# gpcv-liujin/Deep3D_Aerial

Hardware: AMD Instinct MI355X
Metric: cost-volume Mvoxels/s (5v x 384D) (higher is better)
Workload: dtype f32; 1 GPU; config 2: fused homography-warp + variance, 5 views x 384 planes, features 32x688x464 fp32 (2752x1856 image at 1/4 res), one reference view per step per GPU

## Files before the change

### deep3d_aerial_amd/csrc/planesweep_tiled.hip

```cpp
#include "common.h"

#include <hip/hip_fp16.h>

#include "sweep_params.h"
#include "sweep_device.h"

#include <cstdlib>

namespace d3d {

namespace {

constexpr int TW = 32;
#ifndef D3D_NSUB
#define D3D_NSUB 4
#endif
#ifndef D3D_NLOADW
#define D3D_NLOADW 4
#endif
constexpr int DEFAULT_NSUB = D3D_NSUB;
constexpr int DEFAULT_NLOADW = D3D_NLOADW;
constexpr int DEFAULT_NPIXW = 2;
constexpr int DSEG_MAX = 128;
constexpr int MAXSTEPS = 64;
constexpr int PFD = 2;
constexpr int LDS_PIPE = 1;
constexpr int NCAND = 4;
constexpr int MAXRECTS = 512;
constexpr int RING_RW_QUANT = 8;
constexpr int RING_RH_QUANT = 2;
template <int STRIDE>
__host__ __device__ __forceinline__ int ring_row_floats(int RW) {
    const int n = (RW + 1) * STRIDE;
    return ((n - 32 + 63) & ~63) + 32;
}

#ifdef D3D_EXPERIMENTS
#define D3D_STAMPS 1
#else
#define D3D_STAMPS 0
#endif
#define D3D_CLOCK() (D3D_STAMPS ? clock64() : 0ll)

struct TiledArgs {
    int ngroups;
    int dseg;
    int cap_floats;
    int nseg;
    int tiles_x, tiles_y;
    int tall;
    const float* cl;
    unsigned long long* tstats;
    unsigned* stats;
};

template <int CW, int NSRC>
struct Lds {
    static constexpr int STRIDE = CW + 4;
    static constexpr int ZERO = 0;
    static constexpr int PMIN = 2 * STRIDE;
    static constexpr int PMAX = PMIN + DSEG_MAX;
    static constexpr int HDR = PMAX + DSEG_MAX;
    static constexpr int VT = HDR + 32;
    static constexpr int PLAN = VT + 8 * NSRC;
    static constexpr int SST = PLAN + MAXSTEPS * NSRC * 8;
    static constexpr int STOT = SST + MAXSTEPS + 4;
    static constexpr int RECTS = ((STOT + MAXSTEPS + 3) / 4) * 4;
    static constexpr int DATA = RECTS + (MAXRECTS + 1) * 4;
};

__device__ __forceinline__ int posmod(int a, int n) {
    int r = a % n;
    return r < 0 ? r + n : r;
}


struct RingView {
    int RW, RH;
    int rowb;
    int base;
};

template <int STRIDE>
__device__ __forceinline__ TapL geo_ring(const Ray& r, float tx, float ty, float tz, float d, float umax, float vmax, int kx, int ky,
                                         const RingView& R) {
    const float px = __fadd_rn(__fmul_rn(r.rx, d), tx);
    const float py = __fadd_rn(__fmul_rn(r.ry, d), ty);
    const float pz = __fadd_rn(__fmul_rn(r.rz, d), tz);
    const float iz = __builtin_amdgcn_rcpf(pz);
    const float u0 = px * iz, v0 = py * iz;
    float u = fmaf(fmaf(-u0, pz, px), iz, u0);
    float v = fmaf(fmaf(-v0, pz, py), iz, v0);
    u = __builtin_amdgcn_fmed3f(u, -1.0f, umax);
    v = __builtin_amdgcn_fmed3f(v, -1.0f, vmax);
    const float fu = floorf(u), fv = floorf(v);
    const float ax = u - fu, ay = v - fv;
    const float bx = (fu + 1.0f) - u, by = (fv + 1.0f) - v;
    TapL t;
    t.nw = bx * by;
    t.ne = ax * by;
    t.sw = bx * ay;
// ... 238 lines not shown
                vmin = fminf(vmin, v); vmax = fmaxf(vmax, v);
            }
            int wx0 = max((int)floorf(umin - 0.0625f), -1);
            int wy0 = max((int)floorf(vmin - 0.0625f), -1);
            int wx1 = min((int)floorf(umax + 0.0625f) + 1, w + 1);
            int wy1 = min((int)floorf(vmax + 0.0625f) + 1, h + 1);
            int ww = max(wx1 - wx0 + 1, 0), wh = max(wy1 - wy0 + 1, 0);
            if (vsel >= p.n_src) { wx0 = -1; wy0 = -1; ww = 2; wh = 2; ok = true; }
            if (!act) { ww = 0; wh = 0; ok = true; }
            int ux = ww, uy = wh;
            {
                const int qx0 = __shfl_up(wx0, 1), qy0 = __shfl_up(wy0, 1);
                const int qw = __shfl_up(ww, 1), qh = __shfl_up(wh, 1);
                if (lane > 0 && act && qw > 0 && ww > 0) {
                    ux = max(wx0 + ww, qx0 + qw) - min(wx0, qx0);
                    uy = max(wy0 + wh, qy0 + qh) - min(wy0, qy0);
                }
            }
            const int RWc = max(wave_maxi(ux), 1), RHc = max(wave_maxi(uy), 1);
            const int badc = (__any(!ok) || !feasible) ? 1 : 0;
            int* e = ldsi + CT + ((cand * NSRC + vsel) * 64 + lane) * 4;
            e[0] = wx0; e[1] = wy0; e[2] = ww; e[3] = wh;
            if (lane == 0) {
                int* hd = ldsi + CHD + (cand * NSRC + vsel) * 4;
                hd[0] = RWc; hd[1] = RHc; hd[2] = badc; hd[3] = nstepc;
            }
        }
    };
    constexpr int NCAND1 = NCAND - 1;
    for (int wk = wave; wk < NCAND1 * NSRC; wk += NWAVES) candidate_windows(wk / NSRC, wk % NSRC);
    __syncthreads();
    const long long t_p1 = D3D_CLOCK();
    auto plan_tables = [&](int cbeg, int cend) {
        int mode = 0, sp_sel = NSUB, nsteps_sel = (nplanes + NSUB - 1) / NSUB;
        for (int cand = cbeg; cand < cend && !mode; ++cand) {
            const int nsteps = ldsi[CHD + (cand * NSRC) * 4 + 3];
            const bool act = lane < nsteps;
            int wx0[NSRC], wy0[NSRC], ww[NSRC], wh[NSRC], RW[NSRC], RH[NSRC];
            int bad = 0, total = 0, totalq = 0;
            int RWq[NSRC], RHq[NSRC];
#pragma unroll
            for (int i = 0; i < NSRC; ++i) {
                const int* hd = ldsi + CHD + (cand * NSRC + i) * 4;
                RW[i] = hd[0]; RH[i] = hd[1]; bad |= hd[2];
                RWq[i] = (RW[i] + RING_RW_QUANT - 1) / RING_RW_QUANT * RING_RW_QUANT;
                RHq[i] = (RH[i] + RING_RH_QUANT - 1) / RING_RH_QUANT * RING_RH_QUANT;
                total += ring_row_floats<STRIDE>(RW[i]) * (RH[i] + 1);
                totalq += ring_row_floats<STRIDE>(RWq[i]) * (RHq[i] + 1);
            }
            if (totalq <= a.cap_floats) {
                total = totalq;
#pragma unroll
                for (int i = 0; i < NSRC; ++i) { RW[i] = RWq[i]; RH[i] = RHq[i]; }
            }
            if (bad || total > a.cap_floats) continue;
#pragma unroll
            for (int i = 0; i < NSRC; ++i) {
                const int* e = ldsi + CT + ((cand * NSRC + i) * 64 + lane) * 4;
                wx0[i] = e[0]; wy0[i] = e[1]; ww[i] = e[2]; wh[i] = e[3];
            }
            if (!bad && total <= a.cap_floats) {
                mode = 1;
                sp_sel = cand_planes(cand);
                nsteps_sel = nsteps;
                int base = L::DATA;
                int oxv[NSRC], oyv[NSRC], basev[NSRC];
                bool dims_ok = true;
#pragma unroll
                for (int i = 0; i < NSRC; ++i) {
                    const int cx0 = __shfl(wx0[i], 0), cy0 = __shfl(wy0[i], 0);
                    oxv[i] = posmod(wx0[i] - cx0, RW[i]);
                    oyv[i] = posmod(wy0[i] - cy0, RH[i]);
                    basev[i] = base;
                    dims_ok = dims_ok && RW[i] < 256 && RH[i] < 256;
                    if (act) {
                        int* e = ldsi + L::PLAN + (lane * NSRC + i) * 8;
                        e[0] = wx0[i]; e[1] = wy0[i]; e[2] = ww[i]; e[3] = wh[i];
                        e[4] = oxv[i];
                        e[5] = oyv[i];
                        e[6] = oxv[i] - wx0[i];
                        e[7] = oyv[i] - wy0[i];
                    }
                    if (lane == 0) {
                        ldsi[L::HDR + 4 + 4 * i + 0] = RW[i];
                        ldsi[L::HDR + 4 + 4 * i + 1] = RH[i];
                        ldsi[L::HDR + 4 + 4 * i + 2] = base;
                        ldsi[L::HDR + 4 + 4 * i + 3] = RW[i] | (RH[i] << 8) | ((base >> 2) << 16);
                        if constexpr (VIEW_MAJOR) {
                            const float* __restrict__ M = p.proj34 + 12 * min(i, p.n_src - 1);
                            const bool dummy = i >= p.n_src;
                            lds[L::VT + 8 * i + 0] = dummy ? -1.0f : M[3];
                            lds[L::VT + 8 * i + 1] = dummy ? -1.0f : M[7];
                            lds[L::VT + 8 * i + 2] = dummy ? 1.0f : M[11];
                            lds[L::VT + 8 * i + 3] = 0.0f;
                            ldsi[L::VT + 8 * i + 4] = RW[i];
                            ldsi[L::VT + 8 * i + 5] = RH[i];
                            ldsi[L::VT + 8 * i + 6] = ring_row_floats<STRIDE>(RW[i]) * 4;
                            ldsi[L::VT + 8 * i + 7] = lds_base_bytes(lds) + 4 * base;
                        }
                    }
                    base += ring_row_floats<STRIDE>(RW[i]) * (RH[i] + 1);
                }
                int cnt[NSRC][4], rx[NSRC][4], ry[NSRC][4], rwid[NSRC][4], nel[NSRC][4];
                int npos = 0;
#pragma unroll
                for (int i = 0; i < NSRC; ++i) {
                    const int xa = wx0[i], xb = wx0[i] + ww[i] - 1, ya = wy0[i], yb = wy0[i] + wh[i] - 1;
                    const int pxa = __shfl_up(wx0[i], 1), pya = __shfl_up(wy0[i], 1);
                    const int pxb = pxa + __shfl_up(ww[i], 1) - 1, pyb = pya + __shfl_up(wh[i], 1) - 1;
                    int ix0 = 1, ix1 = 0, iy0 = 1, iy1 = 0;
                    if (lane > 0) { ix0 = max(xa, pxa); ix1 = min(xb, pxb); iy0 = max(ya, pya); iy1 = min(yb, pyb); }
                    const bool ov = (ix0 <= ix1) && (iy0 <= iy1);
                    int rh_[4];
                    rx[i][0] = xa;      ry[i][0] = ya;      rwid[i][0] = (ov ? ix0 - 1 : xb) - xa + 1; rh_[0] = wh[i];
                    rx[i][1] = ix1 + 1; ry[i][1] = ya;      rwid[i][1] = ov ? xb - ix1 : 0;             rh_[1] = wh[i];
                    rx[i][2] = ix0;     ry[i][2] = ya;      rwid[i][2] = ov ? ix1 - ix0 + 1 : 0;        rh_[2] = ov ? iy0 - ya : 0;
                    rx[i][3] = ix0;     ry[i][3] = iy1 + 1; rwid[i][3] = ov ? ix1 - ix0 + 1 : 0;        rh_[3] = ov ? yb - iy1 : 0;
#pragma unroll
                    for (int r = 0; r < 4; ++r) {
                        nel[i][r] = act ? max(rwid[i][r], 0) * max(rh_[r], 0) : 0;
                        cnt[i][r] = (nel[i][r] + 63) >> 6;
                        npos += nel[i][r];
                    }
                }
                int nrect = 0;
#pragma unroll
                for (int i = 0; i < NSRC; ++i)
#pragma unroll
                    for (int r = 0; r < 4; ++r) nrect += cnt[i][r] > 0 ? 1 : 0;
                int incl = nrect;
#pragma unroll
                for (int sft = 1; sft < 64; sft <<= 1) {
                    int o = __shfl_up(incl, sft);
                    if (lane >= sft) incl += o;
                }
                const int total_rects = __shfl(incl, 63);
                if (total_rects > MAXRECTS || !dims_ok || __any(npos > 0xffff) || w > 0xfff0 || h > 0xfff0) {
                    mode = 0;
                } else {
                    int idx = incl - nrect;
                    if (act) ldsi[L::SST + lane] = idx;
                    if (lane == nsteps - 1) ldsi[L::SST + nsteps] = incl;
                    int pstart = 0;
#pragma unroll
                    for (int i = 0; i < NSRC; ++i)
#pragma unroll
                        for (int r = 0; r < 4; ++r)
                            if (cnt[i][r] > 0) {
                                int* e = ldsi + L::RECTS + 4 * idx;
                                e[0] = (rx[i][r] + 1) | ((ry[i][r] + 1) << 16);
                                e[1] = rwid[i][r] | (i << 12) | (pstart << 16);
                                e[2] = nel[i][r];
                                e[3] = (rx[i][r] - wx0[i] + oxv[i]) | ((ry[i][r] - wy0[i] + oyv[i]) << 16);
                                pstart += nel[i][r];
                                ++idx;
                            }
                    if (act) ldsi[L::STOT + lane] = pstart;
                }
            }
        }
        if (lane == 0) {
            ldsi[L::HDR + 0] = mode;
            ldsi[L::HDR + 1] = sp_sel;
            ldsi[L::HDR + 2] = nsteps_sel;
        }
    };
    if (wave == 0) plan_tables(0, NCAND1);
    __syncthreads();
    if (rfl(ldsi[L::HDR + 0]) == 0) {
        __syncthreads();
        for (int wk = wave; wk < NSRC; wk += NWAVES) candidate_windows(NCAND1, wk);
        __syncthreads();
        if (wave == 0) plan_tables(NCAND1, NCAND);
        __syncthreads();
    }
    if (D3D_STAMPS && a.tstats && tid == 0) {
        const long long t_p2 = clock64();
        atomicAdd(a.tstats + 16, (unsigned long long)(t_range - t_start));
        atomicAdd(a.tstats + 17, (unsigned long long)(t_p1 - t_range));
        atomicAdd(a.tstats + 18, (unsigned long long)(t_p2 - t_p1));
    }
    const int ring = rfl(ldsi[L::HDR + 0]);
    const int SP = rfl(ldsi[L::HDR + 1]);
    const int nsteps = rfl(ldsi[L::HDR + 2]);
    if (D3D_STAMPS && a.stats && tid == 0) {
        atomicAdd(a.stats + (ring ? 0 : 1), 1u);
        atomicAdd(a.stats + 2, (unsigned)SP);
        atomicAdd(a.stats + 3, (unsigned)nsteps);
        if (ring) {
            unsigned tot = 0;
            for (int i = 0; i < NSRC; ++i) tot += (ldsi[L::HDR + 4 + 4 * i] + 1) * (ldsi[L::HDR + 5 + 4 * i] + 1);
            atomicAdd(a.stats + 4, tot);
        }
    }
    struct Item {
        const float* g;
        int meta;
        int geo;
    };
    long long fdelta[NSRC];
#pragma unroll
    for (int i = 0; i < NSRC; ++i) {
        const long long d0 = reinterpret_cast<long long>(p.feats[1]);
        const long long di = reinterpret_cast<long long>(p.feats[i + 1]);
        fdelta[i] = (i < p.n_src) ? di - d0 : 0;
    }
    auto item = [&](int el, int Tn, int rb, const int (&pst16)[MAXRS]) -> Item {
        Item I;
        const bool live = el < Tn;
        int ridx = rb - 1;
#pragma unroll
        for (int rr = 0; rr < MAXRS; ++rr) ridx += (pst16[rr] <= el) ? 1 : 0;
        ridx = max(ridx, rb);
        const int* e = ldsi + L::RECTS + 4 * ridx;
        const int e0 = e[0], e1 = e[1], e6 = e[3];
        const int rx = (e0 & 0xffff) - 1, ry = (e0 >> 16) - 1;
        const int rwid = e1 & 0xfff, vi = (e1 >> 12) & 0xf, pst = (unsigned)e1 >> 16;
        const int e7 = ldsi[L::HDR + 4 + 4 * vi + 3];
        const int RWv = e7 & 0xff, RHv = (e7 >> 8) & 0xff, bs = (e7 >> 16) << 2;
        const int pos = el - pst;
        const int cy = (int)(((float)pos + 0.5f) * __builtin_amdgcn_rcpf((float)max(rwid, 1)));
        const int cx = pos - cy * rwid;
        const int sx = rx + cx, sy = ry + cy;
        const bool ok = live && ((unsigned)sx < (unsigned)w) && ((unsigned)sy < (unsigned)h);
        long long dsel = 0;
#pragma unroll
        for (int i = 1; i < NSRC; ++i) dsel = (vi == i) ? fdelta[i] : dsel;
        if (a.cl)
            I.g = a.cl + ((size_t)(vi * a.ngroups + grp) * plane + (size_t)(ok ? sy * w + sx : 0)) * CW;
        else
            I.g = reinterpret_cast<const float*>(reinterpret_cast<const char*>(p.feats[1]) + dsel) + (size_t)c0 * plane +
                  (ok ? sy * w + sx : 0);
        unsigned c = (unsigned)((e6 & 0xffff) + cx), r = (unsigned)((e6 >> 16) + cy);
        c = min(c, c - (unsigned)RWv);
        r = min(r, r - (unsigned)RHv);
        const int dst = bs + (int)r * ring_row_floats<STRIDE>(RWv) + (int)c * STRIDE;
        I.meta = live ? (dst | (ok ? 1 << 20 : 0) | (c == 0 ? 1 << 21 : 0) | (r == 0 ? 1 << 22 : 0)) : -1;
        I.geo = e7 & 0xffff;
        return I;
    };
    auto put = [&](int meta, int geo, int q, f4 v) {
        if (meta >= 0) {
            const int dst = (meta & 0xfffff) + 4 * q;
            const int RWv = geo & 0xff, RHv = geo >> 8;
            const int dupc = (meta >> 21) & 1 ? RWv * STRIDE : 0;
            const int dupr = (meta >> 22) & 1 ? RHv * ring_row_floats<STRIDE>(RWv) : 0;
            f4 x = (meta >> 20) & 1 ? v : (f4){0, 0, 0, 0};
            *reinterpret_cast<f4*>(lds + dst) = x;
            if (dupc) *reinterpret_cast<f4*>(lds + dst + dupc) = x;
            if (dupr) *reinterpret_cast<f4*>(lds + dst + dupr) = x;
            if (dupc && dupr) *reinterpret_cast<f4*>(lds + dst + dupc + dupr) = x;
        }
    };
    constexpr bool ONE_RECT = NPIXW <= 2;
    struct Rects {
        int psv, d0, d1, d3, d7;
    };
    const bool small32 = plane <= (size_t)0xffffffffu / (size_t)(CH * 4 > 64 ? CH * 4 : 64);
    f4 pf[PFD][Q];
    int pmeta[PFD], pgeo[PFD];
    int pkind[PFD];
    auto write_round = [&]() {
#pragma unroll
        for (int j = 0; j < PFD; ++j) {
            if (pkind[j] == 0) {
                if (pmeta[j] >= 0) {
#pragma unroll
                    for (int q = 0; q < Q; ++q) *reinterpret_cast<f4*>(lds + pmeta[j] + 4 * q) = pf[j][q];
                }
            } else {
#pragma unroll
                for (int q = 0; q < Q; ++q) put(pmeta[j], pgeo[j], q, pf[j][q]);
            }
        }
    };
    const bool ltiming = D3D_STAMPS && a.tstats != nullptr && lw == 0;
    long long lt_issue = 0, lt_write = 0, lt_bar = 0;
    auto stage = [&](int k, int sw, int snw) {
        const int rb = rfl(ldsi[L::SST + k]), re = rfl(ldsi[L::SST + k + 1]);
        const int Tn = rfl(ldsi[L::STOT + k]);
        const int nitems = (Tn + 63) >> 6;
        Rects R;
        {
            const bool have = lane < re - rb;
            const int* e = ldsi + L::RECTS + 4 * (rb + min(lane, MAXRS - 1));
            R.d1 = e[1];
            R.psv = have ? (int)((unsigned)R.d1 >> 16) : 0x7fffffff;
            if constexpr (ONE_RECT) {
                R.d0 = e[0]; R.d3 = e[3];
                R.d7 = ldsi[L::HDR + 4 + 4 * (have ? (R.d1 >> 12) & 0xf : 0) + 3];
            } else {
                R.d0 = R.d3 = R.d7 = 0;
            }
        }
        const int psv = R.psv;
        int pst16[MAXRS];
#pragma unroll
        for (int rr = 0; rr < MAXRS; ++rr) pst16[rr] = __builtin_amdgcn_readlane(psv, rr);
        unsigned n_items = 0, n_one = 0, n_plain = 0, n_in = 0, n_nodup = 0, n_idle = 0;
        for (int it0 = sw; it0 < nitems; it0 += snw * PFD) {
            long long tq1 = 0, tq2 = 0;
            if (ltiming) tq1 = clock64();
#pragma unroll
            for (int j = 0; j < PFD; ++j) {
                const int it = it0 + snw * j;
                int meta = -1, geo = 0, kind = 0;
                f4 v[Q];
                if (it < nitems) {
                    const int el0 = it * 64;
                    const int nlive = min(Tn - el0, 64);
                    const bool one = ONE_RECT && __ballot(psv > el0 && psv < el0 + nlive) == 0ull;
                    if (D3D_STAMPS) { ++n_items; n_one += one ? 1 : 0; }
                    if (one && small32) {
                        const int rsel = max(__popcll(__ballot(psv <= el0)) - 1, 0);
                        const int e0 = __builtin_amdgcn_readlane(R.d0, rsel), e1 = __builtin_amdgcn_readlane(R.d1, rsel);
                        const int e6 = __builtin_amdgcn_readlane(R.d3, rsel), e7 = __builtin_amdgcn_readlane(R.d7, rsel);
                        const int rx = (e0 & 0xffff) - 1, ry = (e0 >> 16) - 1;
                        const int rwid = e1 & 0xfff, vi = (e1 >> 12) & 0xf, pst = (int)((unsigned)e1 >> 16);
// ... 10 lines not shown
                        const int sx = rx + cx, sy = ry + cy;
                        unsigned c = (unsigned)(oc + cx), r = (unsigned)(orow + cy);
                        c = min(c, c - (unsigned)RWv);
                        r = min(r, r - (unsigned)RHv);
                        const int dst = bs + (int)__umul24(r, (unsigned)ring_row_floats<STRIDE>(RWv)) + (int)__umul24(c, (unsigned)STRIDE);
                        bool ok = live;
                        if (inside && !dups) {
                            meta = live ? dst : -1;
                        } else {
                            if (!inside) ok = live && ((unsigned)sx < (unsigned)w) && ((unsigned)sy < (unsigned)h);
                            meta = live ? (dst | (ok ? 1 << 20 : 0) | (c == 0 ? 1 << 21 : 0) | (r == 0 ? 1 << 22 : 0)) : -1;
                            geo = e7 & 0xffff;
                            kind = 1;
                        }
                        if (D3D_STAMPS) { n_plain += kind == 0 ? 1 : 0; n_in += inside ? 1 : 0; n_nodup += dups ? 0 : 1; }
                        const unsigned soff = ok ? __umul24((unsigned)sy, (unsigned)w) + (unsigned)sx : 0u;
                        if (a.cl) {
                            const char* gb = reinterpret_cast<const char*>(a.cl + (size_t)(vi * a.ngroups + grp) * plane * CW);
                            const f4* __restrict__ g = reinterpret_cast<const f4*>(gb + (size_t)(soff * (unsigned)(CW * 4)));
#pragma unroll
                            for (int q = 0; q < Q; ++q) v[q] = g[q];
                        } else if (!F16) {
                            long long dsel = 0;
#pragma unroll
                            for (int i = 1; i < NSRC; ++i) dsel = (vi == i) ? fdelta[i] : dsel;
                            const char* gb = reinterpret_cast<const char*>(p.feats[1]) + dsel + (size_t)c0 * plane * 4;
#pragma unroll
                            for (int q = 0; q < Q; ++q)
#pragma unroll
                                for (int kk = 0; kk < 4; ++kk)
                                    v[q][kk] = *reinterpret_cast<const float*>(gb + (size_t)(4 * q + kk) * plane * 4 + (size_t)(soff * 4u));
                        }
                    } else {
                        Item I = item(el0 + lane, Tn, rb, pst16);
                        if (a.cl) {
#pragma unroll
                            for (int q = 0; q < Q; ++q) v[q] = reinterpret_cast<const f4*>(I.g)[q];
                        } else if (!F16) {
#pragma unroll
                            for (int q = 0; q < Q; ++q) {
                                const float* __restrict__ g = I.g + (size_t)(4 * q) * plane;
                                v[q][0] = g[0];
                                v[q][1] = g[plane];
                                v[q][2] = g[2 * plane];
                                v[q][3] = g[3 * plane];
                            }
                        }
                        meta = I.meta;
                        geo = I.geo;
                        kind = 1;
                    }
                } else if (D3D_STAMPS) {
                    ++n_idle;
                }
                pmeta[j] = meta;
                pgeo[j] = geo;
                pkind[j] = kind;
#pragma unroll
                for (int q = 0; q < Q; ++q) pf[j][q] = v[q];
            }
            if (ltiming) { tq2 = clock64(); lt_issue += tq2 - tq1; }
            write_round();
            if (ltiming) lt_write += clock64() - tq2;
        }
        if (D3D_STAMPS && a.stats && lane == 0) {
            atomicAdd(a.stats + 5, n_items);
            atomicAdd(a.stats + 6, n_one);
// ... 74 lines not shown
        } else {
#pragma unroll
            for (int k = 0; k < 4; ++k) {
                store_sbase(ob, pixb, o[k]);
                ob += cstride_b;
            }
        }
    };
    auto accumulate = [&](f4& s, f4& qq, float& pair_acc, const f4& val, int q, int i) {
        if (MODE == MODE_VARIANCE) {
            const f2 vl = lo2(val), vh = hi2(val);
            s = cat2(lo2(s) + vl, hi2(s) + vh);
            qq = cat2(pk_fma(vl, vl, lo2(qq)), pk_fma(vh, vh, hi2(qq)));
        } else if (MODE == MODE_WEIGHTED) {
#pragma unroll
            for (int k = 0; k < 4; ++k) s[k] = fmaf(val[k] * r[F16 ? 0 : q][k], vw[i], s[k]);
        } else if (MODE == MODE_PAIR) {
#pragma unroll
            for (int k = 0; k < 4; ++k) pair_acc = fmaf(r[F16 ? 0 : q][k], val[k], pair_acc);
        } else {
            s = val;
        }
    };

    const bool timing = D3D_STAMPS && a.tstats != nullptr && wave == 0;
    const bool wtiming = D3D_STAMPS && a.tstats != nullptr;
    long long t_ww = 0;
    long long t_w = 0, t_w0 = 0, t_c = 0, t_mark = 0;
    if (timing) { t_mark = clock64(); if (lane == 0) atomicAdd(a.tstats + 0, (unsigned long long)(t_mark - t_start)); }
    int kx[NSRC], ky[NSRC];
    int plan_adr = 0;
    auto load_step = [&](int k) {
        if constexpr (VIEW_MAJOR) {
            plan_adr = lds_base_bytes(lds) + 4 * (L::PLAN + (ring ? k : 0) * NSRC * 8);
            return;
        }
#pragma unroll
        for (int i = 0; i < NSRC; ++i) {
            const int* e = ldsi + L::PLAN + ((ring ? k : 0) * NSRC + i) * 8;
            kx[i] = rfl(e[6]);
            ky[i] = rfl(e[7]);
        }
    };
    auto sweep_plane = [&](const int dl_) {
            const int d = ds + dl_;
            float dv;
            if (p.depth_mode == D3D_DEPTH_PER_PIXEL) {
                float t = p.depth[(size_t)d * plane + pix];
                dv = valid ? t : 1.0f;
            } else if (p.depth_mode == D3D_DEPTH_AFFINE) {
                dv = __fadd_rn(aff_lo, __fmul_rn((float)d, aff_step));
            } else {
                dv = lds[L::PMIN + dl_];
            }
            unsigned long long ob = OUTCL ? uniform64(reinterpret_cast<unsigned short*>(p.out) +
                                                      (p.out_cl == 2 ? ((size_t)d * (p.C / 8) + c0 / 8) * plane * 8 : (size_t)d * plane * p.C + c0))
                                          : uniform64(reinterpret_cast<T*>(p.out) + (p.plane_major ? (size_t)d * p.C + c0 : (size_t)c0 * D + d) * plane);
            float pair_acc = 0.0f;
            if (!valid) return;

            if constexpr (VIEW_MAJOR) {
                float sa[Q][CPC], qa[Q][CPC];
#pragma unroll
                for (int q = 0; q < Q; ++q)
#pragma unroll
                    for (int k = 0; k < CPC; ++k) {
                        const float rv = F16 ? rh[F16 ? q : 0][F16 ? k : 0] : r[F16 ? 0 : q][F16 ? 0 : k];
                        sa[q][k] = (MODE == MODE_VARIANCE) ? rv : 0.0f;
                        qa[q][k] = rv * rv;
                    }
                auto accumulate_vm = [&](const float (&val)[CPC], int q, int i) {
#pragma unroll
                    for (int k = 0; k < CPC; k += 2) {
                        const f2 v = {val[k], val[k + 1]};
                        if (MODE == MODE_VARIANCE) {
                            const f2 sn = (f2){sa[q][k], sa[q][k + 1]} + v;
                            const f2 qn = pk_fma(v, v, (f2){qa[q][k], qa[q][k + 1]});
                            sa[q][k] = sn[0]; sa[q][k + 1] = sn[1];
                            qa[q][k] = qn[0]; qa[q][k + 1] = qn[1];
                        } else {
                            sa[q][k] = fmaf(v[0] * r[F16 ? 0 : q][F16 ? 0 : k], vw[i], sa[q][k]);
                            sa[q][k + 1] = fmaf(v[1] * r[F16 ? 0 : q][F16 ? 0 : k + 1], vw[i], sa[q][k + 1]);
                        }
                    }
                };
                if (ring) {
                    const int vt_adr = lds0 + 4 * L::VT;
                    auto geometry = [&](int i) -> TapL {
                        typedef int i4v __attribute__((ext_vector_type(4)));
                        typedef int i2v __attribute__((ext_vector_type(2)));
                        const f4 tv = *(volatile lds_f4_ptr)(unsigned)(vt_adr + 32 * i);
                        const i4v rv = *(volatile __attribute__((address_space(3))) const i4v*)(unsigned)(vt_adr + 32 * i + 16);
                        const i2v kk = *(volatile __attribute__((address_space(3))) const i2v*)(unsigned)(plan_adr + 32 * i + 24);
                        RingView R;
                        R.RW = rv[0]; R.RH = rv[1]; R.rowb = rv[2]; R.base = rv[3];
                        return geo_ring<STRIDE>(ray[i], tv[0], tv[1], tv[2], dv, umax, vmax, kk[0], kk[1], R);
                    };
                    auto fetch = [&](const TapL& g, int q, f4 (&dst)[4]) {
                        dst[0] = lds_read4_abs(g.a0 + q * 16);
                        dst[1] = lds_read4_abs(g.a0 + q * 16 + STRIDE * 4);
                        dst[2] = lds_read4_abs(g.a1 + q * 16);
                        dst[3] = lds_read4_abs(g.a1 + q * 16 + STRIDE * 4);
                    };
                    f4 tp[2][4];
                    TapL gc = geometry(0);
                    fetch(gc, 0, tp[0]);
#pragma unroll
                    for (int i = 0; i < NSRC; ++i) {
                        __builtin_amdgcn_sched_barrier(0);
                        TapL gn = gc;
                        if (i + 1 < NSRC) gn = geometry(i + 1);
#pragma unroll
                        for (int q = 0; q < Q; ++q) {
                            const int u = i * Q + q;
                            if (q + 1 < Q) fetch(gc, q + 1, tp[(u + 1) & 1]);
                            else if (i + 1 < NSRC) fetch(gn, 0, tp[(u + 1) & 1]);
                            f4 (&c)[4] = tp[u & 1];
                            asm volatile("" : "+v"(c[3]));
                            float val[CPC];
                            if constexpr (F16) {
                                const float tw[4] = {gc.nw, gc.ne, gc.sw, gc.se};
#pragma unroll
                                for (int k = 0; k < CPC; ++k) val[k] = 0.0f;
#pragma unroll
                                for (int tp_ = 0; tp_ < 4; ++tp_) {
#pragma unroll
// ... 127 lines not shown
            for (int dl_ = wave / NPIXW; dl_ < nplanes; dl_ += NW) sweep_plane(dl_);
            __syncthreads();
            continue;
        }
        stage(0, wave, NWAVES);
        for (int k = 0; k < nsteps; ++k) {
            long long ta = 0;
            if (timing) ta = clock64();
            long long tw0 = 0;
            if (wtiming) tw0 = clock64();
            __syncthreads();
            if (wtiming && k > 0) t_ww += clock64() - tw0;
            if (timing) { t_mark = clock64(); t_w += t_mark - ta; if (k == 0) t_w0 = t_mark - ta; }
            load_step(k);

            for (int j = 0; sub + NSUB * j < SP; ++j) {
                const int dl_ = k * SP + sub + NSUB * j;
                if (dl_ >= nplanes) break;
                sweep_plane(dl_);
            }
            if (timing) t_c += clock64() - t_mark;
            if constexpr (NLOADW == 0) {
                if (k + 1 < nsteps) stage(k + 1, wave, NWAVES);
            }
        }
        __syncthreads();
        if (timing) t_mark = clock64();
    }
    if (wtiming && lane == 0) atomicAdd(a.tstats + 8 + wave, (unsigned long long)t_ww);
    if (timing && lane == 0) {
        atomicAdd(a.tstats + 1, (unsigned long long)t_w);
        atomicAdd(a.tstats + 5, (unsigned long long)t_w0);
        atomicAdd(a.tstats + 3, (unsigned long long)t_c);
        atomicAdd(a.tstats + 4, (unsigned long long)(clock64() - t_start));
    }
}

struct PackArgs {
    const void* src[D3D_MAX_VIEWS];
};
template <int CH, typename T>
__global__ __launch_bounds__(256) void pack_channel_last_kernel(PackArgs pa, int ngroups, long plane, float* __restrict__ out) {
    constexpr int CW = CH * (int)sizeof(T) / 4, Q = CW / 4, CPC = 16 / (int)sizeof(T);
    const long t = (long)blockIdx.x * 256 + threadIdx.x;
    const long pos = t / Q;
    const int q = (int)(t - pos * Q);
    if (pos >= plane) return;
    const int vg = blockIdx.y;
    const int v = vg / ngroups, g = vg - v * ngroups;
    const T* __restrict__ s = reinterpret_cast<const T*>(pa.src[v]) + ((size_t)g * CH + CPC * q) * plane + pos;
    f4 x;
    if (sizeof(T) == 4) {
        const float* __restrict__ sf = reinterpret_cast<const float*>(s);
        x[0] = sf[0]; x[1] = sf[plane]; x[2] = sf[2 * plane]; x[3] = sf[3 * plane];
    } else {
        const unsigned short* __restrict__ sh = reinterpret_cast<const unsigned short*>(s);
        unsigned wd[4];
#pragma unroll
        for (int k = 0; k < 4; ++k) wd[k] = (unsigned)sh[(2 * k) * plane] | ((unsigned)sh[(2 * k + 1) * plane] << 16);
        x = __builtin_bit_cast(f4, (uint4){wd[0], wd[1], wd[2], wd[3]});
    }
    reinterpret_cast<f4*>(out + ((size_t)vg * plane + pos) * CW)[q] = x;
}

__global__ void zero_first_cells_kernel(float* __restrict__ out, int cells, size_t pitch, int cw) {
    for (int i = threadIdx.x; i < cells * cw; i += blockDim.x) out[(size_t)(i / cw) * pitch + i % cw] = 0.0f;
}
// ... 62 lines not shown
#endif
    segments(p.D, (long)a.tiles_x * a.tiles_y * a.ngroups, a.dseg, a.nseg);
    const long col_tiles = a.tall ? (long)(a.tiles_x - 1) * a.tiles_y + (a.tiles_y + 1) / 2 : (long)a.tiles_x * a.tiles_y;
    const long nblk = col_tiles * a.nseg;
    if (nblk > 0x7fffffffL) return D3D_ERR_UNSUPPORTED;
    a.stats = nullptr;
    a.tstats = nullptr;
    a.cl = nullptr;
    {
        bool use_cl = wants_channel_last(p.D, (int)sizeof(T));
#ifdef D3D_EXPERIMENTS
        if (const char* e = getenv("D3D_TILED_CL")) use_cl = atoi(e) != 0;
#endif
        const size_t bytes = (size_t)NSRC * p.C * p.h * p.w * sizeof(T);
        if (use_cl && p.workspace && p.workspace_bytes >= bytes) {
            PackArgs pa = {};
            for (int i = 0; i < p.n_src; ++i) pa.src[i] = p.feats[i + 1];
            const long plane = (long)p.h * p.w;
            hipLaunchKernelGGL((pack_channel_last_kernel<CH, T>), dim3((unsigned)ceil_div(plane * (CW / 4), 256), p.n_src * a.ngroups),
                               dim3(256), 0, stream, pa, a.ngroups, plane, reinterpret_cast<float*>(p.workspace));
            D3D_LAUNCH_CHECK("pack_channel_last_kernel launch");
            if (p.n_src < NSRC) {
                hipLaunchKernelGGL(zero_first_cells_kernel, dim3(1), dim3(256), 0, stream,
                                   reinterpret_cast<float*>(p.workspace) + (size_t)p.n_src * a.ngroups * plane * CW,
                                   (NSRC - p.n_src) * a.ngroups, (size_t)plane * CW, CW);
                D3D_LAUNCH_CHECK("zero_first_cells_kernel launch");
            }
            a.cl = reinterpret_cast<const float*>(p.workspace);
        }
        if (sizeof(T) == 2 && !a.cl) return D3D_ERR_UNSUPPORTED;
    }
#ifdef D3D_EXPERIMENTS
    if (getenv("D3D_TILED_STATS")) {
        (void)hipMalloc(&a.stats, 12 * sizeof(unsigned) + 24 * sizeof(unsigned long long));
        (void)hipMemset(a.stats, 0, 12 * sizeof(unsigned) + 24 * sizeof(unsigned long long));
        a.tstats = reinterpret_cast<unsigned long long*>(a.stats + 12);
    }
#endif
    hipLaunchKernelGGL(kern, dim3((unsigned)nblk), dim3(THREADSK), LDS_BYTES, stream, p, a);
    D3D_LAUNCH_CHECK("sweep_tiled_kernel launch");
#ifdef D3D_EXPERIMENTS
    if (a.stats) {
        unsigned hs[12];
        unsigned long long ht[24];
        (void)hipMemcpy(hs, a.stats, sizeof(hs), hipMemcpyDeviceToHost);
        (void)hipMemcpy(ht, a.tstats, sizeof(ht), hipMemcpyDeviceToHost);
        fprintf(stderr, "[d3d tiled timing] per-WG mean cycles: compute wave 0: prologue %.0f | barrier wait %.0f (initial window %.0f) | compute %.0f | total %.0f || loader 0: barrier wait %.0f | decode+issue %.0f | wait+write %.0f\n",
                ht[0] / (double)nblk, ht[1] / (double)nblk, ht[5] / (double)nblk, ht[3] / (double)nblk, ht[4] / (double)nblk,
                ht[2] / (double)nblk, ht[6] / (double)nblk, ht[7] / (double)nblk);
        fprintf(stderr, "[d3d tiled timing] prologue phases: depth range %.0f | candidate windows %.0f | plan tables %.0f (rest: per-lane constants)\n",
                ht[16] / (double)nblk, ht[17] / (double)nblk, ht[18] / (double)nblk);
        fprintf(stderr, "[d3d tiled timing] barrier wait after the first, per compute wave (pixel rows, depth sub-range):");
        for (int wv = 0; wv < NPIXK * NSUBK; ++wv) fprintf(stderr, " %.0f", ht[8 + wv] / (double)nblk);
        fprintf(stderr, "\n");
        fprintf(stderr, "[d3d tiled stats] CH=%d elem=%d wgs=%ld ring=%u fallback=%u mean_step_planes=%.2f mean_steps=%.2f mean_ring_positions=%.0f (cap %d) dseg=%d\n",
                CH, (int)sizeof(T), nblk, hs[0], hs[1], hs[2] / (double)nblk, hs[3] / (double)nblk, hs[0] ? hs[4] / (double)hs[0] : 0.0,
                a.cap_floats / L::STRIDE, a.dseg);
        fprintf(stderr, "[d3d tiled stats] staging items per workgroup (all channel groups): %.1f | inside one rectangle %.1f (inside the image %.1f, clear of ring column 0 and row 0 %.1f, both %.1f) | slots with no item left %.1f\n",
                hs[5] / (double)nblk, hs[6] / (double)nblk, hs[8] / (double)nblk, hs[9] / (double)nblk, hs[7] / (double)nblk, hs[10] / (double)nblk);
        (void)hipFree(a.stats);
    }
#endif
    return D3D_OK;
}

static int group_channels(int C, int n_src, int elem_bytes) {
    int cg = (n_src > 4 && elem_bytes == 4) ? 8 : (C >= 16 ? 16 : C);
#ifdef D3D_EXPERIMENTS
    if (const char* e = getenv("D3D_TILED_CG")) cg = atoi(e);
#endif
    if (cg != 8 && cg != 16 && cg != 32) cg = 8;
    while (C % cg) cg >>= 1;
    return cg;
}

template <int MODE, int NSRC>
static int launch_ch(const SweepParams& p, hipStream_t stream) {
    const int cg = (MODE == MODE_PAIR) ? p.C : group_channels(p.C, p.n_src, 4);
    bool shallow = p.D <= SHALLOW_PLANES && cg == 8;
#ifdef D3D_EXPERIMENTS
    if (const char* e = getenv("D3D_TILED_SHALLOW")) shallow = shallow && atoi(e) != 0;
#endif
    if constexpr (MODE == MODE_VARIANCE) {
        if (p.out_cl) {
            if constexpr (SHALLOW_PLANES > 0) {
                if (shallow) return launch_one<MODE, NSRC, 8, float, true, true>(p, stream);
            }
            switch (cg) {
                case 16: return launch_one<MODE, NSRC, 16, float, true>(p, stream);
                case 8: return launch_one<MODE, NSRC, 8, float, true>(p, stream);
            }
            return D3D_ERR_UNSUPPORTED;
// ... 77 lines not shown
```

Measured before the change: 22000 Mvoxels/s.

## Compact LDS plan tables so larger ring buffers fit in shared memory

Shrinks each per-step plan entry from 8 words to 2 (only the ring offsets are kept) and sizes the step, total and rectangle tables from the actual step and rectangle counts rather than worst-case maxima. Table offsets now go into header slots and are read back by the loader waves. The freed LDS lets candidates with more planes per step, or the quantized ring sizes, pass the capacity check, so fewer workgroups fall back to smaller steps or the gather path. In exchange, the rectangle enumeration moves ahead of the capacity check and table addresses are now runtime values, which adds a few LDS reads per stage; it also adds extra experiment-only stats counters.

```diff
diff --git a/deep3d_aerial_amd/csrc/planesweep_tiled.hip b/deep3d_aerial_amd/csrc/planesweep_tiled.hip
--- a/deep3d_aerial_amd/csrc/planesweep_tiled.hip
+++ b/deep3d_aerial_amd/csrc/planesweep_tiled.hip
@@ -26,6 +26,11 @@
 constexpr int PFD = 2;
 constexpr int LDS_PIPE = 1;
 constexpr int NCAND = 4;
+#ifndef D3D_RING_COMPACT
+#define D3D_RING_COMPACT 1
+#endif
+constexpr bool RING_COMPACT = D3D_RING_COMPACT != 0;
+constexpr int PLAN_WORDS = RING_COMPACT ? 2 : 8;
 constexpr int MAXRECTS = 512;
 constexpr int RING_RW_QUANT = 8;
 constexpr int RING_RH_QUANT = 2;
@@ -63,10 +68,21 @@
     static constexpr int HDR = PMAX + DSEG_MAX;
     static constexpr int VT = HDR + 32;
     static constexpr int PLAN = VT + 8 * NSRC;
-    static constexpr int SST = PLAN + MAXSTEPS * NSRC * 8;
+    static constexpr int SST = PLAN + MAXSTEPS * NSRC * PLAN_WORDS;
     static constexpr int STOT = SST + MAXSTEPS + 4;
     static constexpr int RECTS = ((STOT + MAXSTEPS + 3) / 4) * 4;
     static constexpr int DATA = RECTS + (MAXRECTS + 1) * 4;
+    static constexpr int H_CAND = HDR + 3, H_SST = HDR + 28, H_STOT = HDR + 29, H_RECTS = HDR + 30;
+    static __device__ __forceinline__ int tables(int nsteps, int nrects, int& sst, int& stot, int& rects) {
+        if constexpr (!RING_COMPACT) {
+            sst = SST; stot = STOT; rects = RECTS;
+            return DATA;
+        }
+        sst = PLAN + nsteps * NSRC * PLAN_WORDS;
+        stot = sst + nsteps + 1;
+        rects = (stot + nsteps + 3) & ~3;
+        return rects + (nrects + 1) * 4;
+    }
 };
 
 __device__ __forceinline__ int posmod(int a, int n) {
@@ -371,9 +387,10 @@
     __syncthreads();
     const long long t_p1 = D3D_CLOCK();
     auto plan_tables = [&](int cbeg, int cend) {
-        int mode = 0, sp_sel = NSUB, nsteps_sel = (nplanes + NSUB - 1) / NSUB;
+        int mode = 0, sp_sel = NSUB, nsteps_sel = (nplanes + NSUB - 1) / NSUB, cand_sel = NCAND, tab_sel = 0;
+        const int lds_floats = a.cap_floats + L::DATA;
         for (int cand = cbeg; cand < cend && !mode; ++cand) {
-            const int nsteps = ldsi[CHD + (cand * NSRC) * 4 + 3];
+            const int nsteps = rfl(ldsi[CHD + (cand * NSRC) * 4 + 3]);
             const bool act = lane < nsteps;
             int wx0[NSRC], wy0[NSRC], ww[NSRC], wh[NSRC], RW[NSRC], RH[NSRC];
             int bad = 0, total = 0, totalq = 0;
@@ -381,44 +398,79 @@
 #pragma unroll
             for (int i = 0; i < NSRC; ++i) {
                 const int* hd = ldsi + CHD + (cand * NSRC + i) * 4;
-                RW[i] = hd[0]; RH[i] = hd[1]; bad |= hd[2];
+                RW[i] = rfl(hd[0]); RH[i] = rfl(hd[1]); bad |= rfl(hd[2]);
                 RWq[i] = (RW[i] + RING_RW_QUANT - 1) / RING_RW_QUANT * RING_RW_QUANT;
                 RHq[i] = (RH[i] + RING_RH_QUANT - 1) / RING_RH_QUANT * RING_RH_QUANT;
                 total += ring_row_floats<STRIDE>(RW[i]) * (RH[i] + 1);
                 totalq += ring_row_floats<STRIDE>(RWq[i]) * (RHq[i] + 1);
             }
-            if (totalq <= a.cap_floats) {
-                total = totalq;
-#pragma unroll
-                for (int i = 0; i < NSRC; ++i) { RW[i] = RWq[i]; RH[i] = RHq[i]; }
-            }
-            if (bad || total > a.cap_floats) continue;
+            int sst, stot, rects;
+            if (bad || L::tables(nsteps, 0, sst, stot, rects) + total > lds_floats) continue;
 #pragma unroll
             for (int i = 0; i < NSRC; ++i) {
                 const int* e = ldsi + CT + ((cand * NSRC + i) * 64 + lane) * 4;
                 wx0[i] = e[0]; wy0[i] = e[1]; ww[i] = e[2]; wh[i] = e[3];
             }
-            if (!bad && total <= a.cap_floats) {
+            {
+                int rx[NSRC][4], ry[NSRC][4], rwid[NSRC][4], nel[NSRC][4];
+                int npos = 0;
+#pragma unroll
+                for (int i = 0; i < NSRC; ++i) {
+                    const int xa = wx0[i], xb = wx0[i] + ww[i] - 1, ya = wy0[i], yb = wy0[i] + wh[i] - 1;
+                    const int pxa = __shfl_up(wx0[i], 1), pya = __shfl_up(wy0[i], 1);
+                    const int pxb = pxa + __shfl_up(ww[i], 1) - 1, pyb = pya + __shfl_up(wh[i], 1) - 1;
+                    int ix0 = 1, ix1 = 0, iy0 = 1, iy1 = 0;
+                    if (lane > 0) { ix0 = max(xa, pxa); ix1 = min(xb, pxb); iy0 = max(ya, pya); iy1 = min(yb, pyb); }
+                    const bool ov = (ix0 <= ix1) && (iy0 <= iy1);
+                    int rh_[4];
+                    rx[i][0] = xa;      ry[i][0] = ya;      rwid[i][0] = (ov ? ix0 - 1 : xb) - xa + 1; rh_[0] = wh[i];
+                    rx[i][1] = ix1 + 1; ry[i][1] = ya;      rwid[i][1] = ov ? xb - ix1 : 0;             rh_[1] = wh[i];
+                    rx[i][2] = ix0;     ry[i][2] = ya;      rwid[i][2] = ov ? ix1 - ix0 + 1 : 0;        rh_[2] = ov ? iy0 - ya : 0;
+                    rx[i][3] = ix0;     ry[i][3] = iy1 + 1; rwid[i][3] = ov ? ix1 - ix0 + 1 : 0;        rh_[3] = ov ? yb - iy1 : 0;
+#pragma unroll
+                    for (int r = 0; r < 4; ++r) {
+                        nel[i][r] = act ? max(rwid[i][r], 0) * max(rh_[r], 0) : 0;
+                        npos += nel[i][r];
+                    }
+                }
+                int nrect = 0;
+#pragma unroll
+                for (int i = 0; i < NSRC; ++i)
+#pragma unroll
+                    for (int r = 0; r < 4; ++r) nrect += nel[i][r] > 0 ? 1 : 0;
+                int incl = nrect;
+#pragma unroll
+                for (int sft = 1; sft < 64; sft <<= 1) {
+                    int o = __shfl_up(incl, sft);
+                    if (lane >= sft) incl += o;
+                }
+                const int total_rects = __shfl(incl, 63);
+                int base = L::tables(nsteps, total_rects, sst, stot, rects);
+                if (base + totalq <= lds_floats) {
+                    total = totalq;
+#pragma unroll
+                    for (int i = 0; i < NSRC; ++i) { RW[i] = RWq[i]; RH[i] = RHq[i]; }
+                }
+                if (base + total > lds_floats) continue;
+                bool dims_ok = true;
+#pragma unroll
+                for (int i = 0; i < NSRC; ++i) dims_ok = dims_ok && RW[i] < 256 && RH[i] < 256;
+                if ((!RING_COMPACT && total_rects > MAXRECTS) || !dims_ok || __any(npos > 0xffff) || w > 0xfff0 || h > 0xfff0) continue;
                 mode = 1;
                 sp_sel = cand_planes(cand);
                 nsteps_sel = nsteps;
-                int base = L::DATA;
-                int oxv[NSRC], oyv[NSRC], basev[NSRC];
-                bool dims_ok = true;
+                cand_sel = cand;
+                tab_sel = base - L::PLAN;
+                int oxv[NSRC], oyv[NSRC];
 #pragma unroll
                 for (int i = 0; i < NSRC; ++i) {
                     const int cx0 = __shfl(wx0[i], 0), cy0 = __shfl(wy0[i], 0);
                     oxv[i] = posmod(wx0[i] - cx0, RW[i]);
                     oyv[i] = posmod(wy0[i] - cy0, RH[i]);
-                    basev[i] = base;
-                    dims_ok = dims_ok && RW[i] < 256 && RH[i] < 256;
                     if (act) {
-                        int* e = ldsi + L::PLAN + (lane * NSRC + i) * 8;
-                        e[0] = wx0[i]; e[1] = wy0[i]; e[2] = ww[i]; e[3] = wh[i];
-                        e[4] = oxv[i];
-                        e[5] = oyv[i];
-                        e[6] = oxv[i] - wx0[i];
-                        e[7] = oyv[i] - wy0[i];
+                        int* e = ldsi + L::PLAN + (lane * NSRC + i) * PLAN_WORDS;
+                        e[PLAN_WORDS - 2] = oxv[i] - wx0[i];
+                        e[PLAN_WORDS - 1] = oyv[i] - wy0[i];
                     }
                     if (lane == 0) {
                         ldsi[L::HDR + 4 + 4 * i + 0] = RW[i];
@@ -440,53 +492,17 @@
                     }
                     base += ring_row_floats<STRIDE>(RW[i]) * (RH[i] + 1);
                 }
-                int cnt[NSRC][4], rx[NSRC][4], ry[NSRC][4], rwid[NSRC][4], nel[NSRC][4];
-                int npos = 0;
-#pragma unroll
-                for (int i = 0; i < NSRC; ++i) {
-                    const int xa = wx0[i], xb = wx0[i] + ww[i] - 1, ya = wy0[i], yb = wy0[i] + wh[i] - 1;
-                    const int pxa = __shfl_up(wx0[i], 1), pya = __shfl_up(wy0[i], 1);
-                    const int pxb = pxa + __shfl_up(ww[i], 1) - 1, pyb = pya + __shfl_up(wh[i], 1) - 1;
-                    int ix0 = 1, ix1 = 0, iy0 = 1, iy1 = 0;
-                    if (lane > 0) { ix0 = max(xa, pxa); ix1 = min(xb, pxb); iy0 = max(ya, pya); iy1 = min(yb, pyb); }
-                    const bool ov = (ix0 <= ix1) && (iy0 <= iy1);
-                    int rh_[4];
-                    rx[i][0] = xa;      ry[i][0] = ya;      rwid[i][0] = (ov ? ix0 - 1 : xb) - xa + 1; rh_[0] = wh[i];
-                    rx[i][1] = ix1 + 1; ry[i][1] = ya;      rwid[i][1] = ov ? xb - ix1 : 0;             rh_[1] = wh[i];
-                    rx[i][2] = ix0;     ry[i][2] = ya;      rwid[i][2] = ov ? ix1 - ix0 + 1 : 0;        rh_[2] = ov ? iy0 - ya : 0;
-                    rx[i][3] = ix0;     ry[i][3] = iy1 + 1; rwid[i][3] = ov ? ix1 - ix0 + 1 : 0;        rh_[3] = ov ? yb - iy1 : 0;
-#pragma unroll
-                    for (int r = 0; r < 4; ++r) {
-                        nel[i][r] = act ? max(rwid[i][r], 0) * max(rh_[r], 0) : 0;
-                        cnt[i][r] = (nel[i][r] + 63) >> 6;
-                        npos += nel[i][r];
-                    }
-                }
-                int nrect = 0;
-#pragma unroll
-                for (int i = 0; i < NSRC; ++i)
-#pragma unroll
-                    for (int r = 0; r < 4; ++r) nrect += cnt[i][r] > 0 ? 1 : 0;
-                int incl = nrect;
-#pragma unroll
-                for (int sft = 1; sft < 64; sft <<= 1) {
-                    int o = __shfl_up(incl, sft);
-                    if (lane >= sft) incl += o;
-                }
-                const int total_rects = __shfl(incl, 63);
-                if (total_rects > MAXRECTS || !dims_ok || __any(npos > 0xffff) || w > 0xfff0 || h > 0xfff0) {
-                    mode = 0;
-                } else {
+                {
                     int idx = incl - nrect;
-                    if (act) ldsi[L::SST + lane] = idx;
-                    if (lane == nsteps - 1) ldsi[L::SST + nsteps] = incl;
+                    if (act) ldsi[sst + lane] = idx;
+                    if (lane == nsteps - 1) ldsi[sst + nsteps] = incl;
                     int pstart = 0;
 #pragma unroll
                     for (int i = 0; i < NSRC; ++i)
 #pragma unroll
                         for (int r = 0; r < 4; ++r)
-                            if (cnt[i][r] > 0) {
-                                int* e = ldsi + L::RECTS + 4 * idx;
+                            if (nel[i][r] > 0) {
+                                int* e = ldsi + rects + 4 * idx;
                                 e[0] = (rx[i][r] + 1) | ((ry[i][r] + 1) << 16);
                                 e[1] = rwid[i][r] | (i << 12) | (pstart << 16);
                                 e[2] = nel[i][r];
@@ -494,7 +510,12 @@
                                 pstart += nel[i][r];
                                 ++idx;
                             }
-                    if (act) ldsi[L::STOT + lane] = pstart;
+                    if (act) ldsi[stot + lane] = pstart;
+                    if (lane == 0) {
+                        ldsi[L::H_SST] = sst;
+                        ldsi[L::H_STOT] = stot;
+                        ldsi[L::H_RECTS] = rects;
+                    }
                 }
             }
         }
@@ -502,6 +523,8 @@
             ldsi[L::HDR + 0] = mode;
             ldsi[L::HDR + 1] = sp_sel;
             ldsi[L::HDR + 2] = nsteps_sel;
+            ldsi[L::H_CAND] = cand_sel;
+            if (D3D_STAMPS) ldsi[L::HDR + 31] = tab_sel;
         }
     };
     if (wave == 0) plan_tables(0, NCAND1);
@@ -531,6 +554,8 @@
             for (int i = 0; i < NSRC; ++i) tot += (ldsi[L::HDR + 4 + 4 * i] + 1) * (ldsi[L::HDR + 5 + 4 * i] + 1);
             atomicAdd(a.stats + 4, tot);
         }
+        atomicAdd(a.stats + 12 + min(ldsi[L::H_CAND], NCAND), 1u);
+        atomicAdd(a.stats + 11, (unsigned)ldsi[L::HDR + 31]);
     }
     struct Item {
         const float* g;
@@ -544,14 +569,14 @@
         const long long di = reinterpret_cast<long long>(p.feats[i + 1]);
         fdelta[i] = (i < p.n_src) ? di - d0 : 0;
     }
-    auto item = [&](int el, int Tn, int rb, const int (&pst16)[MAXRS]) -> Item {
+    auto item = [&](int el, int Tn, int rb, int rects, const int (&pst16)[MAXRS]) -> Item {
         Item I;
         const bool live = el < Tn;
         int ridx = rb - 1;
 #pragma unroll
         for (int rr = 0; rr < MAXRS; ++rr) ridx += (pst16[rr] <= el) ? 1 : 0;
         ridx = max(ridx, rb);
-        const int* e = ldsi + L::RECTS + 4 * ridx;
+        const int* e = ldsi + rects + 4 * ridx;
         const int e0 = e[0], e1 = e[1], e6 = e[3];
         const int rx = (e0 & 0xffff) - 1, ry = (e0 >> 16) - 1;
         const int rwid = e1 & 0xfff, vi = (e1 >> 12) & 0xf, pst = (unsigned)e1 >> 16;
@@ -616,13 +641,15 @@
     const bool ltiming = D3D_STAMPS && a.tstats != nullptr && lw == 0;
     long long lt_issue = 0, lt_write = 0, lt_bar = 0;
     auto stage = [&](int k, int sw, int snw) {
-        const int rb = rfl(ldsi[L::SST + k]), re = rfl(ldsi[L::SST + k + 1]);
-        const int Tn = rfl(ldsi[L::STOT + k]);
+        const int sst = RING_COMPACT ? rfl(ldsi[L::H_SST]) : L::SST, stot = RING_COMPACT ? rfl(ldsi[L::H_STOT]) : L::STOT;
+        const int rects = RING_COMPACT ? rfl(ldsi[L::H_RECTS]) : L::RECTS;
+        const int rb = rfl(ldsi[sst + k]), re = rfl(ldsi[sst + k + 1]);
+        const int Tn = rfl(ldsi[stot + k]);
         const int nitems = (Tn + 63) >> 6;
         Rects R;
         {
             const bool have = lane < re - rb;
-            const int* e = ldsi + L::RECTS + 4 * (rb + min(lane, MAXRS - 1));
+            const int* e = ldsi + rects + 4 * (rb + min(lane, MAXRS - 1));
             R.d1 = e[1];
             R.psv = have ? (int)((unsigned)R.d1 >> 16) : 0x7fffffff;
             if constexpr (ONE_RECT) {
@@ -699,7 +726,7 @@
                                     v[q][kk] = *reinterpret_cast<const float*>(gb + (size_t)(4 * q + kk) * plane * 4 + (size_t)(soff * 4u));
                         }
                     } else {
-                        Item I = item(el0 + lane, Tn, rb, pst16);
+                        Item I = item(el0 + lane, Tn, rb, rects, pst16);
                         if (a.cl) {
 #pragma unroll
                             for (int q = 0; q < Q; ++q) v[q] = reinterpret_cast<const f4*>(I.g)[q];
@@ -840,14 +867,14 @@
     int plan_adr = 0;
     auto load_step = [&](int k) {
         if constexpr (VIEW_MAJOR) {
-            plan_adr = lds_base_bytes(lds) + 4 * (L::PLAN + (ring ? k : 0) * NSRC * 8);
+            plan_adr = lds_base_bytes(lds) + 4 * (L::PLAN + (ring ? k : 0) * NSRC * PLAN_WORDS + PLAN_WORDS - 2);
             return;
         }
 #pragma unroll
         for (int i = 0; i < NSRC; ++i) {
-            const int* e = ldsi + L::PLAN + ((ring ? k : 0) * NSRC + i) * 8;
-            kx[i] = rfl(e[6]);
-            ky[i] = rfl(e[7]);
+            const int* e = ldsi + L::PLAN + ((ring ? k : 0) * NSRC + i) * PLAN_WORDS;
+            kx[i] = rfl(e[PLAN_WORDS - 2]);
+            ky[i] = rfl(e[PLAN_WORDS - 1]);
         }
     };
     auto sweep_plane = [&](const int dl_) {
@@ -899,7 +926,7 @@
                         typedef int i2v __attribute__((ext_vector_type(2)));
                         const f4 tv = *(volatile lds_f4_ptr)(unsigned)(vt_adr + 32 * i);
                         const i4v rv = *(volatile __attribute__((address_space(3))) const i4v*)(unsigned)(vt_adr + 32 * i + 16);
-                        const i2v kk = *(volatile __attribute__((address_space(3))) const i2v*)(unsigned)(plan_adr + 32 * i + 24);
+                        const i2v kk = *(volatile __attribute__((address_space(3))) const i2v*)(unsigned)(plan_adr + 4 * PLAN_WORDS * i);
                         RingView R;
                         R.RW = rv[0]; R.RH = rv[1]; R.rowb = rv[2]; R.base = rv[3];
                         return geo_ring<STRIDE>(ray[i], tv[0], tv[1], tv[2], dv, umax, vmax, kk[0], kk[1], R);
@@ -1093,7 +1120,9 @@
         atomicAdd(a.tstats + 1, (unsigned long long)t_w);
         atomicAdd(a.tstats + 5, (unsigned long long)t_w0);
         atomicAdd(a.tstats + 3, (unsigned long long)t_c);
-        atomicAdd(a.tstats + 4, (unsigned long long)(clock64() - t_start));
+        const unsigned long long t_all = (unsigned long long)(clock64() - t_start);
+        atomicAdd(a.tstats + 4, t_all);
+        atomicAdd(a.tstats + 24 + min(ldsi[L::H_CAND], NCAND), t_all);
     }
 }
 
@@ -1222,17 +1251,17 @@
     }
 #ifdef D3D_EXPERIMENTS
     if (getenv("D3D_TILED_STATS")) {
-        (void)hipMalloc(&a.stats, 12 * sizeof(unsigned) + 24 * sizeof(unsigned long long));
-        (void)hipMemset(a.stats, 0, 12 * sizeof(unsigned) + 24 * sizeof(unsigned long long));
-        a.tstats = reinterpret_cast<unsigned long long*>(a.stats + 12);
+        (void)hipMalloc(&a.stats, 20 * sizeof(unsigned) + 32 * sizeof(unsigned long long));
+        (void)hipMemset(a.stats, 0, 20 * sizeof(unsigned) + 32 * sizeof(unsigned long long));
+        a.tstats = reinterpret_cast<unsigned long long*>(a.stats + 20);
     }
 #endif
     hipLaunchKernelGGL(kern, dim3((unsigned)nblk), dim3(THREADSK), LDS_BYTES, stream, p, a);
     D3D_LAUNCH_CHECK("sweep_tiled_kernel launch");
 #ifdef D3D_EXPERIMENTS
     if (a.stats) {
-        unsigned hs[12];
-        unsigned long long ht[24];
+        unsigned hs[20];
+        unsigned long long ht[32];
         (void)hipMemcpy(hs, a.stats, sizeof(hs), hipMemcpyDeviceToHost);
         (void)hipMemcpy(ht, a.tstats, sizeof(ht), hipMemcpyDeviceToHost);
         fprintf(stderr, "[d3d tiled timing] per-WG mean cycles: compute wave 0: prologue %.0f | barrier wait %.0f (initial window %.0f) | compute %.0f | total %.0f || loader 0: barrier wait %.0f | decode+issue %.0f | wait+write %.0f\n",
@@ -1248,6 +1277,15 @@
                 a.cap_floats / L::STRIDE, a.dseg);
         fprintf(stderr, "[d3d tiled stats] staging items per workgroup (all channel groups): %.1f | inside one rectangle %.1f (inside the image %.1f, clear of ring column 0 and row 0 %.1f, both %.1f) | slots with no item left %.1f\n",
                 hs[5] / (double)nblk, hs[6] / (double)nblk, hs[8] / (double)nblk, hs[9] / (double)nblk, hs[7] / (double)nblk, hs[10] / (double)nblk);
+        {
+            fprintf(stderr, "[d3d tiled stats] plan tables %.0f words per workgroup (worst-case layout: %d) | workgroups (mean total cycles) by planes per step:",
+                    hs[11] / (double)nblk, L::DATA - L::PLAN);
+            for (int c = 0; c < NCAND; ++c) {
+                const int sp = c < 3 ? NSUBK * (4 >> c) : max(NSUBK / 2, 1);
+                fprintf(stderr, " %d: %u (%.0f)", sp, hs[12 + c], hs[12 + c] ? ht[24 + c] / (double)hs[12 + c] : 0.0);
+            }
+            fprintf(stderr, " gather: %u (%.0f)\n", hs[12 + NCAND], hs[12 + NCAND] ? ht[24 + NCAND] / (double)hs[12 + NCAND] : 0.0);
+        }
         (void)hipFree(a.stats);
     }
 #endif
```

Result: no change. 22100 Mvoxels/s, median of 6 (+0.5%).
